# willi-menapace/PlayableEnvironments

Hardware: AMD Instinct MI355X
Metric: Mrays/s (higher is better)
Workload: dtype f32; 1 GPU; tennis renderer, 256x256 frame per GPU (rank r renders the frame of seed 1234 + r), 4 objects, 64+128 hierarchical samples/ray (coarse+fine networks), eval - BASELINE.json configs[1]; rays_per_gpu=65536, frames_per_gpu=1, parallelism=frame shard x1

## Files before the change

### playableenvironments_amd/csrc/composite.hip

```cpp
#include "pr_common.h"
#include "composite_dev.h"

namespace pr {

struct CompositeSmem {
    float* tt;
    float* sg;
    float* dm;
    float* wo;
    float* wg;
    float* al;
    float* dv;
    int* sl;
    unsigned int* key;
};

constexpr int MAX_FCHUNK = 4;

__device__ __forceinline__ void transmittance_weights(float* al, int n, int lane) {
    float carry = 1.0f;
    for (int base = 0; base < n; base += 64) {
        const int j = base + lane;
        const float a = (j < n) ? al[j] : 0.f;
        float incl = (j < n) ? __fadd_rn(__fsub_rn(1.0f, a), 1e-10f) : 1.0f;
#pragma unroll
        for (int d = 1; d < 64; d <<= 1) {
            const float o = __shfl_up(incl, d, 64);
            if (lane >= d) incl *= o;
        }
        float excl = __shfl_up(incl, 1, 64);
        if (lane == 0) excl = 1.0f;
        if (j < n) al[j] = a * (carry * excl);
        carry *= __shfl(incl, 63, 64);
    }
}

constexpr int ROWS_IN_FLIGHT = 8;

__device__ __forceinline__ float sigmoid_of(float x) { return 1.0f / (1.0f + expf(-x)); }

template <int CW>
__device__ __forceinline__ void transmittance_weights_block(float* al, int n, float* totals, int wave, int lane) {
    if (CW == 1) {
        transmittance_weights(al, n, lane);
        return;
    }
    const int seg = (((n + CW - 1) / CW) + 63) & ~63;
    const int begin = wave * seg;
    const int end = (begin + seg < n) ? begin + seg : n;
    float carry = 1.0f;
    for (int base = begin; base < end; base += 64) {
        const int j = base + lane;
        const float a = (j < end) ? al[j] : 0.f;
        float incl = (j < end) ? __fadd_rn(__fsub_rn(1.0f, a), 1e-10f) : 1.0f;
#pragma unroll
        for (int d = 1; d < 64; d <<= 1) {
            const float o = __shfl_up(incl, d, 64);
            if (lane >= d) incl *= o;
        }
        float excl = __shfl_up(incl, 1, 64);
        if (lane == 0) excl = 1.0f;
        if (j < end) al[j] = a * (carry * excl);
        carry *= __shfl(incl, 63, 64);
    }
    if (lane == 0) totals[wave] = carry;
    __syncthreads();
    float before = 1.0f;
    for (int w = 0; w < wave; ++w) before *= totals[w];
    if (wave > 0)
        for (int j = begin + lane; j < end; j += 64) al[j] *= before;
    __syncthreads();
}

template <int CW>
__device__ __forceinline__ float block_sum(float v, float* scratch, int wave, int lane) {
    v = wave_sum(v);
    if (CW == 1) return v;
    __syncthreads();
    if (lane == 0) scratch[wave] = v;
    __syncthreads();
    float total = 0.f;
    for (int w = 0; w < CW; ++w) total += scratch[w];
    return total;
}

template <int CW>
__device__ __forceinline__ void store_channel_sums(float (&acc)[MAX_FCHUNK], float* dst, int F, float* scratch, int wave, int lane) {
    if (CW > 1) {
#pragma unroll
        for (int c = 0; c < MAX_FCHUNK; ++c) {
            if (64 * c >= F) break;
            __syncthreads();
            scratch[wave * 64 + lane] = acc[c];
            __syncthreads();
            if (wave == 0)
                for (int w = 1; w < CW; ++w) acc[c] = __fadd_rn(acc[c], scratch[w * 64 + lane]);
        }
    }
    if (wave == 0) {
#pragma unroll
        for (int c = 0; c < MAX_FCHUNK; ++c) {
            const int ch = lane + 64 * c;
            if (ch < F) dst[ch] = acc[c];
        }
    }
}

template <int CW>
__global__ __launch_bounds__(64 * CW) void k_composite(CompositeParams p) {
    extern __shared__ __attribute__((aligned(16))) char raw_smem[];
    constexpr int CT = 64 * CW;
    const int S = p.sort_size;
    CompositeSmem sm;
    const int A = (p.total_positions + 63) & ~63;
    sm.key = reinterpret_cast<unsigned int*>(raw_smem);
    sm.tt = reinterpret_cast<float*>(sm.key + S);
    sm.sg = sm.tt + A;
    sm.dm = sm.sg + A;
    sm.wo = sm.dm + A;
    sm.wg = sm.sg;
    sm.al = sm.wo + A;
    const bool use_div = p.any_divergence != 0;
    sm.dv = use_div ? sm.al + A : nullptr;
    sm.sl = reinterpret_cast<int*>(sm.al + (use_div ? 2 * A : A));
    float* scratch = reinterpret_cast<float*>(sm.sl + A);
    unsigned long long* wide = p.fix_overlaps ? reinterpret_cast<unsigned long long*>(scratch + 4 * 64) : nullptr;

    const int tid = threadIdx.x, lane = tid & 63;
    const int wave = (CW == 1) ? 0 : __builtin_amdgcn_readfirstlane(tid >> 6);
    const long g = blockIdx.x;
    const float* d = p.ray_directions + (size_t)g * 3;
    const float norm = sqrtf(__fadd_rn(__fadd_rn(__fmul_rn(d[0], d[0]), __fmul_rn(d[1], d[1])), __fmul_rn(d[2], d[2])));
    const int PT = p.total_positions;

    {
        int off = 0;
        for (int k = 0; k < p.objects; ++k) {
            const CompositeObject& o = p.obj[k];
            const int P = o.positions;
            const size_t base = (size_t)g * P;
            for (int i = tid; i < P; i += CT) {
                sm.tt[off + i] = o.t[base + i];
                sm.sg[off + i] = o.sigma[base + i];
                sm.sl[off + i] = o.slot[base + i];
                sm.dm[off + i] = o.dispmag ? o.dispmag[base + i] : 0.f;
                if (use_div) sm.dv[off + i] = o.divergence ? fabsf(o.divergence[base + i]) : 0.f;
            }
            off += P;
        }
    }
    __syncthreads();

    for (int round = 0; round * CW < p.objects; ++round) {
        const int k = round * CW + wave;
        const bool mine = k < p.objects;
        int off = 0;
        for (int q = 0; q < k && q < p.objects; ++q) off += p.obj[q].positions;
        const CompositeObject& o = p.obj[mine ? k : 0];
        const int P = mine ? o.positions : 0;
        const size_t base = (size_t)g * P;
        float adiv = 0.f;
        for (int i = lane; i < P; i += 64) {
            const float dt = (i < P - 1) ? __fsub_rn(sm.tt[off + i + 1], sm.tt[off + i]) : 1e10f;
            float raw = sm.sg[off + i];
            if (noise_present(o.noise)) raw = __fadd_rn(raw, noise_normal(o.noise, g, P, i));
            const float a = alpha_of(raw, __fmul_rn(dt, norm));
            sm.al[off + i] = a;
            if (use_div) adiv += a * sm.dv[off + i];
        }
        adiv = wave_sum(adiv);
        __syncthreads();
        if (mine) transmittance_weights(sm.al + off, P, lane);
        __syncthreads();
        float depth = 0.f, opacity = 0.f, dmag = 0.f;
        for (int i = lane; i < P; i += 64) {
            const float w = sm.al[off + i];
            sm.wo[off + i] = w;
            if (o.out.weights) o.out.weights[base + i] = w;
            depth += w * sm.tt[off + i];
            opacity += w;
            dmag += w * sm.dm[off + i];
        }
        depth = wave_sum(depth);
        opacity = wave_sum(opacity);
        dmag = wave_sum(dmag);
        if (mine && lane == 0) {
            if (o.out.depth) o.out.depth[g] = depth;
            if (o.out.opacity) o.out.opacity[g] = opacity;
            if (o.out.disparity) o.out.disparity[g] = disparity_of(depth, opacity);
            if (o.out.integrated_displacements_magnitude) o.out.integrated_displacements_magnitude[g] = dmag / (float)P;
            if (o.out.integrated_divergence) o.out.integrated_divergence[g] = adiv / (float)P;
        }
    }
    __syncthreads();

    if (p.fix_overlaps) {
        int dyn_off0 = 0;
        for (int k = 0; k < p.static_objects; ++k) dyn_off0 += p.obj[k].positions;
        int soff = 0;
        for (int s = 0; s < p.static_objects; ++s) {
            const int Ps = p.obj[s].positions;
            unsigned int masked_bits = 0;
            int doff = dyn_off0;
            for (int dd = p.static_objects; dd < p.objects; ++dd) {
                const float b0 = sm.tt[doff + 0];
                const float b1 = sm.tt[doff + Ps - 1];
                int lo0 = 0, hi0 = Ps;
                while (lo0 < hi0) {
                    const int mid = (lo0 + hi0) >> 1;
                    if (sm.tt[soff + mid] < b0) lo0 = mid + 1; else hi0 = mid;
                }
                int lo1 = 0, hi1 = Ps;
                while (lo1 < hi1) {
                    const int mid = (lo1 + hi1) >> 1;
                    if (sm.tt[soff + mid] < b1) lo1 = mid + 1; else hi1 = mid;
                }
                int m = 0;
                for (int i = tid; i < Ps; i += CT, ++m)
                    if (i >= lo0 && i < lo1) masked_bits |= 1u << m;
                doff += p.obj[dd].positions;
            }
            __syncthreads();
            int m = 0;
            for (int i = tid; i < Ps; i += CT, ++m) {
                if ((masked_bits >> m) & 1u) {
                    sm.tt[soff + i] = 0.f;
                    sm.sg[soff + i] = -10.0f;
                    sm.dm[soff + i] = 0.f;
                    if (use_div) sm.dv[soff + i] = 0.f;
                }
            }
            __syncthreads();
            soff += Ps;
        }
    }

    {
        int counts[PR_MAX_OBJECTS];
        for (int k = 0; k < p.objects; ++k) counts[k] = p.obj[k].positions;
        order_entries(sm.key, sm.tt, counts, p.objects, PT, S, !p.fix_overlaps, tid, CT, wide);
    }

    const size_t gbase = (size_t)g * PT;
    float gdiv = 0.f;
    for (int j = tid; j < PT; j += CT) {
        const int e = (int)sm.key[j];
        float dt = 1e10f;
        if (j < PT - 1) {
            const int en = (int)sm.key[j + 1];
            dt = __fsub_rn(sm.tt[en], sm.tt[e]);
        }
        float raw = sm.sg[e];
        if (noise_present(p.noise_global)) raw = __fadd_rn(raw, noise_normal(p.noise_global, g, PT, j));
        sm.al[j] = alpha_of(raw, __fmul_rn(dt, norm));
        if (use_div) gdiv += sm.al[j] * sm.dv[e];
    }
    __syncthreads();
    transmittance_weights_block<CW>(sm.al, PT, scratch, wave, lane);
    if (CW == 1) __syncthreads();
    {
        float depth = 0.f, opacity = 0.f, dmag = 0.f;
        for (int j = tid; j < PT; j += CT) {
            const int e = (int)sm.key[j];
            const float w = sm.al[j];
            sm.wg[e] = w;
            if (p.global.weights) p.global.weights[gbase + j] = w;
            depth += w * sm.tt[e];
            opacity += w;
            dmag += w * sm.dm[e];
        }
        depth = block_sum<CW>(depth, scratch, wave, lane);
        opacity = block_sum<CW>(opacity, scratch, wave, lane);
        dmag = block_sum<CW>(dmag, scratch, wave, lane);
        if (use_div) gdiv = block_sum<CW>(gdiv, scratch, wave, lane);
        if (tid == 0) {
            if (p.global.depth) p.global.depth[g] = depth;
            if (p.global.opacity) p.global.opacity[g] = opacity;
            if (p.global.disparity) p.global.disparity[g] = disparity_of(depth, opacity);
            if (p.global.integrated_displacements_magnitude)
                p.global.integrated_displacements_magnitude[g] = dmag / (float)PT;
            if (p.global.integrated_divergence) p.global.integrated_divergence[g] = gdiv / (float)PT;
        }
    }
    __syncthreads();

    if (p.geometry) {
        if (p.visibility != nullptr || p.front_object != nullptr) {
            float best = 0.f;
            int front = -1;
            int goff = 0;
            for (int k = 0; k < p.objects; ++k) {
                const int P = p.obj[k].positions;
                float v = 0.f;
                for (int i = tid; i < P; i += CT) v += sm.wg[goff + i];
                v = block_sum<CW>(v, scratch, wave, lane);
                if (tid == 0 && p.visibility != nullptr) as_global(p.visibility)[(size_t)g * p.objects + k] = v;
                if (v > best) {
                    best = v;
                    front = k;
                }
                goff += P;
            }
            if (tid == 0 && p.front_object != nullptr) as_global(p.front_object)[g] = front;
        }
        return;
    }

    const int F = p.F;
    const bool defer = p.pooled != nullptr;
    int* lrow = reinterpret_cast<int*>(sm.key);
    float* lw1 = sm.tt;
    float accg[MAX_FCHUNK];
#pragma unroll
    for (int c = 0; c < MAX_FCHUNK; ++c) accg[c] = 0.f;
    int off = 0;
    for (int k = 0; k < p.objects; ++k) {
        const CompositeObject& o = p.obj[k];
        const int P = o.positions;
        const int part = (((P + CW - 1) / CW) + 63) & ~63;
        const int begin = wave * part;
        const int end = (begin + part < P) ? begin + part : P;
        __syncthreads();
        int count = 0;
        float bare1 = 0.f, bare2 = 0.f;
        for (int base = begin; base < end; base += 64) {
            const int i = base + lane;
            bool take = false;
            int row = -1;
            float w1 = 0.f, w2 = 0.f;
            if (i < end) {
                row = sm.sl[off + i];
                w1 = sm.wo[off + i];
                w2 = sm.wg[off + i];
                take = row >= 0 && (w1 != 0.f || w2 != 0.f);
                if (p.sigmoid && row < 0) {
                    bare1 += w1;
                    bare2 += w2;
                }
            }
            const unsigned long long m = __ballot(take);
            if (take) {
                const int pos = off + begin + count + __popcll(m & ((1ull << lane) - 1ull));
                lrow[pos] = row;
                lw1[pos] = w1;
                sm.al[pos] = w2;
            }
            count += __popcll(m);
        }
        const int* rows_w = lrow + off + begin;
        const float* w1_w = lw1 + off + begin;
        const float* w2_w = sm.al + off + begin;
        float acco[MAX_FCHUNK];
#pragma unroll
        for (int c = 0; c < MAX_FCHUNK; ++c) acco[c] = 0.f;
        int i = 0;
        for (; i + ROWS_IN_FLIGHT <= count; i += ROWS_IN_FLIGHT) {
            float v[ROWS_IN_FLIGHT][MAX_FCHUNK];
#pragma unroll
            for (int u = 0; u < ROWS_IN_FLIGHT; ++u) {
                const float* f = o.feat + (size_t)rows_w[i + u] * F;
#pragma unroll
                for (int c = 0; c < MAX_FCHUNK; ++c) {
                    const int ch = lane + 64 * c;
                    v[u][c] = (ch < F) ? f[ch] : 0.f;
                    if (p.sigmoid) v[u][c] = sigmoid_of(v[u][c]);
                }
            }
#pragma unroll
            for (int u = 0; u < ROWS_IN_FLIGHT; ++u) {
                const float w1 = w1_w[i + u], w2 = w2_w[i + u];
#pragma unroll
                for (int c = 0; c < MAX_FCHUNK; ++c) {
                    acco[c] = __fadd_rn(acco[c], __fmul_rn(w1, v[u][c]));
                    accg[c] = __fadd_rn(accg[c], __fmul_rn(w2, v[u][c]));
                }
            }
        }
        for (; i < count; ++i) {
            const float* f = o.feat + (size_t)rows_w[i] * F;
            const float w1 = w1_w[i], w2 = w2_w[i];
#pragma unroll
            for (int c = 0; c < MAX_FCHUNK; ++c) {
                const int ch = lane + 64 * c;
                float v = (ch < F) ? f[ch] : 0.f;
                if (p.sigmoid) v = sigmoid_of(v);
                acco[c] = __fadd_rn(acco[c], __fmul_rn(w1, v));
                accg[c] = __fadd_rn(accg[c], __fmul_rn(w2, v));
            }
        }
        if (p.sigmoid) {
            bare1 = wave_sum(bare1);
            bare2 = wave_sum(bare2);
#pragma unroll
            for (int c = 0; c < MAX_FCHUNK; ++c) {
                acco[c] = __fadd_rn(acco[c], 0.5f * bare1);
                accg[c] = __fadd_rn(accg[c], 0.5f * bare2);
            }
        }
        if (o.out.integrated_features)
            store_channel_sums<CW>(acco, defer ? p.pooled + ((size_t)(2 * k) * gridDim.x + g) * F : o.out.integrated_features + (size_t)g * F, F,
                                   scratch, wave, lane);
        if (defer) {
            if (p.global.integrated_features || p.decoder.groups > 0)
                store_channel_sums<CW>(accg, p.pooled + ((size_t)(2 * k + 1) * gridDim.x + g) * F, F, scratch, wave, lane);
#pragma unroll
            for (int c = 0; c < MAX_FCHUNK; ++c) accg[c] = 0.f;
        }
        off += P;
    }
    if (defer) return;
    if (p.global.integrated_features) store_channel_sums<CW>(accg, p.global.integrated_features + (size_t)g * F, F, scratch, wave, lane);
    if (p.decoder.groups > 0) {
        if (CW > 1 && !p.global.integrated_features) {
#pragma unroll
            for (int c = 0; c < MAX_FCHUNK; ++c) {
                if (64 * c >= F) break;
                __syncthreads();
                scratch[wave * 64 + lane] = accg[c];
                __syncthreads();
                if (wave == 0)
                    for (int w = 1; w < CW; ++w) accg[c] = __fadd_rn(accg[c], scratch[w * 64 + lane]);
            }
        }
        if (wave == 0) {
            const int frame = (int)(g / p.rays);
            int r = (int)(g - (long)frame * p.rays);
            int grp = 0;
            while (grp < p.decoder.groups - 1 && r >= p.decoder.rays[grp]) r -= p.decoder.rays[grp++];
            const int c0 = p.decoder.channel_begin[grp], c1 = p.decoder.channel_end[grp];
            const size_t cells = (size_t)p.decoder.rays[grp];
            float* map = p.decoder.map[grp] + (size_t)frame * (c1 - c0) * cells + r;
#pragma unroll
            for (int c = 0; c < MAX_FCHUNK; ++c) {
                const int ch = lane + 64 * c;
                if (ch >= c0 && ch < c1 && ch < F) map[(size_t)(ch - c0) * cells] = accg[c];
            }
        }
    }
}

int launch_composite(const CompositeParams& p, hipStream_t s) {
    PR_REQUIRE(p.F <= 64 * MAX_FCHUNK, "output_features %d exceeds %d", p.F, 64 * MAX_FCHUNK);
    PR_REQUIRE(p.sort_size >= p.total_positions && (p.sort_size & (p.sort_size - 1)) == 0, "bad sort size");
    for (int k = 0; k < p.objects; ++k)
        PR_REQUIRE(p.obj[k].positions <= 64 * 32, "positions per ray %d too large for the overlap mask", p.obj[k].positions);
    const size_t lds = (size_t)p.sort_size * 4 + (size_t)((p.total_positions + 63) & ~63) * (p.any_divergence ? 7 : 6) * 4 +
                       sizeof(float) * 4 * 64 + (p.fix_overlaps ? (size_t)p.sort_size * 8 : 0);
    PR_REQUIRE(lds <= 156 * 1024, "too many samples per ray for the compositing kernel (%d)", p.total_positions);
    if (p.decoder.groups > 0) {
        PR_REQUIRE(p.decoder.groups <= PR_MAX_DECODER_GROUPS, "decoder layout: %d groups (max %d)", p.decoder.groups, PR_MAX_DECODER_GROUPS);
        long sum = 0;
        for (int i = 0; i < p.decoder.groups; ++i) {
            PR_REQUIRE(p.decoder.rays[i] > 0 && p.decoder.width[i] > 0 && p.decoder.rays[i] % p.decoder.width[i] == 0,
                       "decoder layout: group %d has %d rays in rows of %d", i, p.decoder.rays[i], p.decoder.width[i]);
            PR_REQUIRE(p.decoder.channel_begin[i] >= 0 && p.decoder.channel_begin[i] < p.decoder.channel_end[i] && p.decoder.channel_end[i] <= (p.pooled ? p.out_features : p.F),
                       "decoder layout: group %d channel range [%d, %d) outside 0..%d", i, p.decoder.channel_begin[i], p.decoder.channel_end[i], p.pooled ? p.out_features : p.F);
            PR_REQUIRE(p.decoder.map[i] != nullptr, "decoder layout: group %d has no map", i);
            sum += p.decoder.rays[i];
        }
        PR_REQUIRE(sum == p.rays, "decoder layout: the groups hold %ld rays, the call has %d", sum, p.rays);
    }
    const long total = (long)p.frames * p.rays;
    ProfileScope scope(1, s);
    if (p.total_positions >= 256) {
        PR_TRY(prepare_kernel(reinterpret_cast<const void*>(&k_composite<4>), 156 * 1024, nullptr));
        hipLaunchKernelGGL(k_composite<4>, dim3((unsigned)total), dim3(256), lds, s, p);
    } else {
        PR_TRY(prepare_kernel(reinterpret_cast<const void*>(&k_composite<1>), 156 * 1024, nullptr));
        hipLaunchKernelGGL(k_composite<1>, dim3((unsigned)total), dim3(64), lds, s, p);
    }
    PR_LAUNCH_CHECK();
    return PR_OK;
}

typedef float f32x16 __attribute__((ext_vector_type(16)));
constexpr int PJ_ROWS = 64;
constexpr int PJ_KMAX = MAX_WIDTH / 2 + 8;
constexpr int PJ_LDA = PJ_KMAX + 4;

__global__ __launch_bounds__(256) void k_project_features(CompositeParams p) {
    __shared__ __attribute__((aligned(16))) float SA[PJ_ROWS * PJ_LDA];
    const int tid = threadIdx.x, lane = tid & 63, r = lane & 31, half = lane >> 5;
    const int wave = __builtin_amdgcn_readfirstlane(tid >> 6);
    const long total = (long)p.frames * p.rays;
    const long row0 = (long)blockIdx.x * PJ_ROWS;
    const int HW = p.F, PK = p.proj_k, F = p.out_features;
    const int nblk = (F + 31) / 32;
    const int k4 = PK >> 2;
    const bool want_global = p.global.integrated_features != nullptr || p.decoder.groups > 0;
    for (int set = 0; set <= p.objects; ++set) {
        const bool global = set == p.objects;
        float* out = global ? p.global.integrated_features : p.obj[set].out.integrated_features;
        if (global ? !want_global : out == nullptr) continue;
        f32x16 acc[2][2];
#pragma unroll
        for (int a = 0; a < 2; ++a)
#pragma unroll
            for (int b = 0; b < 2; ++b)
#pragma unroll
                for (int i = 0; i < 16; ++i) acc[a][b][i] = 0.f;
        const int kfirst = global ? 0 : set, klast = global ? p.objects - 1 : set;
        for (int k = kfirst; k <= klast; ++k) {
            const float* A = p.pooled + ((size_t)(2 * k + (global ? 1 : 0)) * total + row0) * HW;
            __syncthreads();
            for (int idx = tid; idx < PJ_ROWS * k4; idx += 256) {
                const int row = idx / k4, c = (idx - row * k4) * 4;
                float4 v = make_float4(0.f, 0.f, 0.f, 0.f);
                if (row0 + row < total && c < HW) v = *reinterpret_cast<const float4*>(A + (size_t)row * HW + c);
                *reinterpret_cast<float4*>(SA + row * PJ_LDA + c) = v;
            }
            __syncthreads();
            const float* W = p.proj_w[k];
            const float* a0 = SA + r * PJ_LDA + 4 * half;
#pragma unroll
            for (int blk = 0; blk < 2; ++blk) {
                const int cb = wave + 4 * blk;
                if (cb >= nblk) continue;
                const auto* wp = as_global(reinterpret_cast<const f32x4_t*>(W + (size_t)(cb * 32 + r) * PK + 4 * half));
                for (int q = 0; q < k4; q += 2) {
                    const f32x4_t w = wp[q];
                    const float4 x0 = *reinterpret_cast<const float4*>(a0 + 4 * q);
                    const float4 x1 = *reinterpret_cast<const float4*>(a0 + 32 * PJ_LDA + 4 * q);
                    acc[blk][0] = __builtin_amdgcn_mfma_f32_32x32x2f32(x0.x, w.x, acc[blk][0], 0, 0, 0);
                    acc[blk][1] = __builtin_amdgcn_mfma_f32_32x32x2f32(x1.x, w.x, acc[blk][1], 0, 0, 0);
                    acc[blk][0] = __builtin_amdgcn_mfma_f32_32x32x2f32(x0.y, w.y, acc[blk][0], 0, 0, 0);
                    acc[blk][1] = __builtin_amdgcn_mfma_f32_32x32x2f32(x1.y, w.y, acc[blk][1], 0, 0, 0);
                    acc[blk][0] = __builtin_amdgcn_mfma_f32_32x32x2f32(x0.z, w.z, acc[blk][0], 0, 0, 0);
                    acc[blk][1] = __builtin_amdgcn_mfma_f32_32x32x2f32(x1.z, w.z, acc[blk][1], 0, 0, 0);
                    acc[blk][0] = __builtin_amdgcn_mfma_f32_32x32x2f32(x0.w, w.w, acc[blk][0], 0, 0, 0);
                    acc[blk][1] = __builtin_amdgcn_mfma_f32_32x32x2f32(x1.w, w.w, acc[blk][1], 0, 0, 0);
                }
            }
        }
#pragma unroll
        for (int blk = 0; blk < 2; ++blk) {
            const int col = (wave + 4 * blk) * 32 + r;
            if (col >= F) continue;
#pragma unroll
            for (int rb = 0; rb < 2; ++rb) {
#pragma unroll
                for (int i = 0; i < 16; ++i) {
                    const long g = row0 + 32 * rb + (i & 3) + 8 * (i >> 2) + 4 * half;
                    if (g >= total) continue;
                    const float v = acc[blk][rb][i];
                    if (out) out[(size_t)g * F + col] = v;
                    if (global && p.decoder.groups > 0) {
                        const int frame = (int)(g / p.rays);
                        int rr = (int)(g - (long)frame * p.rays);
                        int grp = 0;
                        while (grp < p.decoder.groups - 1 && rr >= p.decoder.rays[grp]) rr -= p.decoder.rays[grp++];
                        const int c0 = p.decoder.channel_begin[grp], c1 = p.decoder.channel_end[grp];
                        const size_t cells = (size_t)p.decoder.rays[grp];
                        float* map = p.decoder.map[grp] + (size_t)frame * (c1 - c0) * cells + rr;
                        if (col >= c0 && col < c1) map[(size_t)(col - c0) * cells] = v;
                    }
                }
            }
        }
    }
}

int launch_projection(const CompositeParams& p, hipStream_t s) {
    PR_REQUIRE(p.pooled != nullptr, "deferred projection without pooled rows");
    PR_REQUIRE(p.proj_k >= p.F && p.proj_k <= PJ_KMAX && (p.proj_k & 7) == 0 && (p.F & 3) == 0, "deferred projection: row of %d floats, K %d",
               p.F, p.proj_k);
    PR_REQUIRE(p.out_features >= 1 && p.out_features <= 256, "deferred projection: output_features %d", p.out_features);
    for (int k = 0; k < p.objects; ++k) PR_REQUIRE(p.proj_w[k] != nullptr, "deferred projection: object %d has no packed matrix", k);
    const long total = (long)p.frames * p.rays;
    ProfileScope scope(1, s);
    hipLaunchKernelGGL(k_project_features, dim3((unsigned)((total + PJ_ROWS - 1) / PJ_ROWS)), dim3(256), 0, s, p);
    PR_LAUNCH_CHECK();
    return PR_OK;
}

}
```

Before: 0.3294 Mrays/s.

## Parallelize feature projection across output sets via grid y dimension

The projection kernel now launches one grid slice per output set (the global set plus each object with integrated features) instead of looping over all sets inside every block. The shared-memory staging loads are restructured so each wave loads several rows into registers before storing them. The next weight vector is prefetched one iteration ahead. Output and decoder-map stores are split into separate loops. This adds parallelism and overlaps memory latency, but it is only one stage of a large renderer.

```diff
diff --git a/playableenvironments_amd/csrc/composite.hip b/playableenvironments_amd/csrc/composite.hip
--- a/playableenvironments_amd/csrc/composite.hip
+++ b/playableenvironments_amd/csrc/composite.hip
@@ -488,10 +488,16 @@
     const int nblk = (F + 31) / 32;
     const int k4 = PK >> 2;
     const bool want_global = p.global.integrated_features != nullptr || p.decoder.groups > 0;
-    for (int set = 0; set <= p.objects; ++set) {
+    {
+        int set = p.objects;
+        if (!want_global || blockIdx.y > 0) {
+            set = 0;
+            for (int wanted = (int)blockIdx.y - (want_global ? 1 : 0); set < p.objects; ++set)
+                if (p.obj[set].out.integrated_features != nullptr && wanted-- == 0) break;
+            if (set == p.objects) return;
+        }
         const bool global = set == p.objects;
         float* out = global ? p.global.integrated_features : p.obj[set].out.integrated_features;
-        if (global ? !want_global : out == nullptr) continue;
         f32x16 acc[2][2];
 #pragma unroll
         for (int a = 0; a < 2; ++a)
@@ -503,11 +509,17 @@
         for (int k = kfirst; k <= klast; ++k) {
             const float* A = p.pooled + ((size_t)(2 * k + (global ? 1 : 0)) * total + row0) * HW;
             __syncthreads();
-            for (int idx = tid; idx < PJ_ROWS * k4; idx += 256) {
-                const int row = idx / k4, c = (idx - row * k4) * 4;
-                float4 v = make_float4(0.f, 0.f, 0.f, 0.f);
-                if (row0 + row < total && c < HW) v = *reinterpret_cast<const float4*>(A + (size_t)row * HW + c);
-                *reinterpret_cast<float4*>(SA + row * PJ_LDA + c) = v;
+            if (lane < k4) {
+                const int c = 4 * lane;
+                f32x4_t v[PJ_ROWS / 4];
+#pragma unroll
+                for (int u = 0; u < PJ_ROWS / 4; ++u) {
+                    const int row = wave + 4 * u;
+                    v[u] = f32x4_t{0.f, 0.f, 0.f, 0.f};
+                    if (row0 + row < total && c < HW) v[u] = *as_global(reinterpret_cast<const f32x4_t*>(A + (size_t)row * HW + c));
+                }
+#pragma unroll
+                for (int u = 0; u < PJ_ROWS / 4; ++u) *reinterpret_cast<f32x4_t*>(SA + (wave + 4 * u) * PJ_LDA + c) = v[u];
             }
             __syncthreads();
             const float* W = p.proj_w[k];
@@ -517,8 +529,10 @@
                 const int cb = wave + 4 * blk;
                 if (cb >= nblk) continue;
                 const auto* wp = as_global(reinterpret_cast<const f32x4_t*>(W + (size_t)(cb * 32 + r) * PK + 4 * half));
+                f32x4_t w_next = wp[0];
                 for (int q = 0; q < k4; q += 2) {
-                    const f32x4_t w = wp[q];
+                    const f32x4_t w = w_next;
+                    w_next = wp[q + 2 < k4 ? q + 2 : q];
                     const float4 x0 = *reinterpret_cast<const float4*>(a0 + 4 * q);
                     const float4 x1 = *reinterpret_cast<const float4*>(a0 + 32 * PJ_LDA + 4 * q);
                     acc[blk][0] = __builtin_amdgcn_mfma_f32_32x32x2f32(x0.x, w.x, acc[blk][0], 0, 0, 0);
@@ -532,32 +546,45 @@
                 }
             }
         }
-#pragma unroll
-        for (int blk = 0; blk < 2; ++blk) {
-            const int col = (wave + 4 * blk) * 32 + r;
-            if (col >= F) continue;
+        const int col0 = wave * 32 + r, col1 = col0 + 4 * 32;
+        if (out) {
 #pragma unroll
             for (int rb = 0; rb < 2; ++rb) {
 #pragma unroll
                 for (int i = 0; i < 16; ++i) {
                     const long g = row0 + 32 * rb + (i & 3) + 8 * (i >> 2) + 4 * half;
                     if (g >= total) continue;
-                    const float v = acc[blk][rb][i];
-                    if (out) out[(size_t)g * F + col] = v;
-                    if (global && p.decoder.groups > 0) {
-                        const int frame = (int)(g / p.rays);
-                        int rr = (int)(g - (long)frame * p.rays);
-                        int grp = 0;
-                        while (grp < p.decoder.groups - 1 && rr >= p.decoder.rays[grp]) rr -= p.decoder.rays[grp++];
-                        const int c0 = p.decoder.channel_begin[grp], c1 = p.decoder.channel_end[grp];
-                        const size_t cells = (size_t)p.decoder.rays[grp];
-                        float* map = p.decoder.map[grp] + (size_t)frame * (c1 - c0) * cells + rr;
-                        if (col >= c0 && col < c1) map[(size_t)(col - c0) * cells] = v;
-                    }
-                }
-            }
-        }
-    }
+                    if (col0 < F) out[(size_t)g * F + col0] = acc[0][rb][i];
+                    if (col1 < F) out[(size_t)g * F + col1] = acc[1][rb][i];
+                }
+            }
+        }
+        if (global && p.decoder.groups > 0) {
+#pragma unroll
+            for (int rb = 0; rb < 2; ++rb) {
+#pragma unroll
+                for (int i = 0; i < 16; ++i) {
+                    const long g = row0 + 32 * rb + (i & 3) + 8 * (i >> 2) + 4 * half;
+                    if (g >= total) continue;
+                    const int frame = (int)(g / p.rays);
+                    int rr = (int)(g - (long)frame * p.rays);
+                    int grp = 0;
+                    while (grp < p.decoder.groups - 1 && rr >= p.decoder.rays[grp]) rr -= p.decoder.rays[grp++];
+                    const int c0 = p.decoder.channel_begin[grp], c1 = p.decoder.channel_end[grp];
+                    const size_t cells = (size_t)p.decoder.rays[grp];
+                    float* map = p.decoder.map[grp] + (size_t)frame * (c1 - c0) * cells + rr;
+                    if (col0 < F && col0 >= c0 && col0 < c1) map[(size_t)(col0 - c0) * cells] = acc[0][rb][i];
+                    if (col1 < F && col1 >= c0 && col1 < c1) map[(size_t)(col1 - c0) * cells] = acc[1][rb][i];
+                }
+            }
+        }
+    }
+}
+
+static int projection_sets(const CompositeParams& p) {
+    int sets = (p.global.integrated_features != nullptr || p.decoder.groups > 0) ? 1 : 0;
+    for (int k = 0; k < p.objects; ++k) sets += p.obj[k].out.integrated_features != nullptr ? 1 : 0;
+    return sets;
 }
 
 int launch_projection(const CompositeParams& p, hipStream_t s) {
@@ -567,8 +594,10 @@
     PR_REQUIRE(p.out_features >= 1 && p.out_features <= 256, "deferred projection: output_features %d", p.out_features);
     for (int k = 0; k < p.objects; ++k) PR_REQUIRE(p.proj_w[k] != nullptr, "deferred projection: object %d has no packed matrix", k);
     const long total = (long)p.frames * p.rays;
+    const int sets = projection_sets(p);
+    if (sets == 0) return PR_OK;
     ProfileScope scope(1, s);
-    hipLaunchKernelGGL(k_project_features, dim3((unsigned)((total + PJ_ROWS - 1) / PJ_ROWS)), dim3(256), 0, s, p);
+    hipLaunchKernelGGL(k_project_features, dim3((unsigned)((total + PJ_ROWS - 1) / PJ_ROWS), (unsigned)sets), dim3(256), 0, s, p);
     PR_LAUNCH_CHECK();
     return PR_OK;
 }
```

New measurement: 0.3316 Mrays/s, median of 6. No clear change (+0.7%).
